# griffin-h/lightcurve_fitting

Hardware: AMD Instinct MI355X
Metric: walker-steps/sec (emcee ensemble) (higher is better)
Workload: dtype f64

## Files before the change

lightcurve_fitting_amd/csrc/lcf_hip.hip:

```cpp
#include <hip/hip_runtime.h>

#include <algorithm>
#include <chrono>
#include <cmath>
#include <cstdio>
#include <cstdlib>
#include <dlfcn.h>
#include <cstring>
#include <mutex>
#include <numeric>
#include <string>
#include <vector>

#include "lcf.h"
#include "lcf_device.h"
#include "lcf_host.h"
#include "lcf_internal.h"
#include "lcf_keys.h"

#ifndef LCF_KPRE
#define LCF_KPRE 4
#endif
#ifndef LCF_KPRE_SOLO
#define LCF_KPRE_SOLO 2
// ... 937 lines not shown
        step_serial<ND>(pb, sm, i, true, threadIdx.x, have_prev, prev_row, have_next, draws, prev_draws, g, mine, sc, nullptr,
                        coef, lprior);
}

template <int ND>
__global__ __launch_bounds__(64) void k_step(const DevProblem pb, const DevSampler sm, int have_prev, long long prev_row,
                                             int have_next, const DrawRec* __restrict__ draws,
                                             const DrawRec* __restrict__ prev_draws, long long g, int lo, int hi,
                                             double* __restrict__ coef, double* __restrict__ lprior) {
    step_body<ND>(pb, sm, blockIdx.x, have_prev, prev_row, have_next, draws, prev_draws, g, lo, hi, coef, lprior);
}

constexpr int kFusedScratch = kNCoef + 2 + kMaxDim + (kMaxDim & 1);

__device__ inline double uniform_f64(double v) {
    const long long b = __double_as_longlong(v);
    const int lo = __builtin_amdgcn_readfirstlane((int)(b & 0xffffffffLL));
    const int hi = __builtin_amdgcn_readfirstlane((int)(b >> 32));
    return __longlong_as_double(((long long)hi << 32) | (unsigned int)lo);
}

template <int ND, int VARIANT, bool THERM>
__global__ __launch_bounds__(kBlock, LCF_WAVES) void k_fused(const DevProblem pb, const DevSampler sm, int have_prev,
                                                  long long prev_row, const DrawRec* __restrict__ draws,
                                                  const DrawRec* __restrict__ prev_draws, long long g, int lo, int hi,
                                                  double* __restrict__ lprior) {
    extern __shared__ __align__(16) unsigned char smem[];
    double* exptab = reinterpret_cast<double*>(smem);
    double* red = exptab + kExpTabSize;
    double2* ltab = reinterpret_cast<double2*>(smem + kLdsHead * sizeof(double));
    const FiltDesc* fdesc = reinterpret_cast<const FiltDesc*>(ltab + pb.n_lds_tab);
    const int itab_at = pb.n_itab_lds > 0
                            ? (int)(kLdsHead * sizeof(double) + (pb.n_lds_tab + kFdD2 * pb.n_filters) * sizeof(double2)) : -1;
    double* sc = reinterpret_cast<double*>(ltab + pb.stage_d2);
    double* sq = sc + kNCoef + 2;
    const int tid = threadIdx.x;
    const int n_own = hi - lo;
    if ((int)blockIdx.x >= n_own * pb.n_parts) {
        const int k = ((int)blockIdx.x - n_own * pb.n_parts) * (kBlock / 64) + (tid >> 6);
        const int slot = k < lo ? k : k + n_own;
        if (slot < sm.n_half)
            step_serial<ND>(pb, sm, slot, true, tid & 63, have_prev, prev_row, 1, draws, prev_draws, g, false, nullptr,
                            nullptr, nullptr, nullptr);
        return;
    }
    const int part = blockIdx.x / n_own, i = lo + blockIdx.x % n_own;
    const bool reddened = pb.model == kShockCooling3;
    if (tid < 64)
        step_serial<ND>(pb, sm, i, part == 0, tid, have_prev, prev_row, 1, draws, prev_draws, g, true, sc, sq, nullptr,
                        lprior);
    else if (!reddened)
        stage_tables<VARIANT, true>(pb, exptab, ltab, 0., tid - 64, kBlock - 64);
    __syncthreads();
    if (sc[kNCoef] == -INFINITY) return;
    double cs[kNCoef];
#pragma unroll
    for (int k = 0; k < kNCoef; ++k) cs[k] = uniform_f64(sc[k]);
    if (reddened) stage_tables<VARIANT, true>(pb, exptab, ltab, cs[6], tid, kBlock);
    if (reddened) __syncthreads();
    double term;
    if constexpr (THERM)
        term = epochs_loop<VARIANT, true>(pb, part, sq, cs, ltab, fdesc, ExpTab{exptab}, tid, itab_at);
    else
        term = points_loop<VARIANT, 0, true, false>(pb, part, 0, sq, cs, nullptr, 0, ltab, fdesc, ExpTab{exptab}, nullptr,
                                                    nullptr, tid, itab_at);
    const double psum = store_part_sum(term, red, sm.part2[g & 1] + (size_t)i * part_stride(pb) + part);
    if (sm.n_peers > 0 && tid == 0) mbox_post(sm, g, i, part, part_stride(pb), psum);
}

__device__ inline unsigned long long* board_entry(unsigned long long* board, const DevSampler& sm, unsigned int tag, int wid,
                                                  int col) {
    return board + 2 * ((((size_t)(tag & (unsigned int)(sm.ring - 1)) * sm.n_walkers) + wid) * board_row_entries(sm.n_dim) + col);
}
#ifndef LCF_EARLY_POST
#define LCF_EARLY_POST 0
#endif
#ifndef LCF_EARLY_LOG
#define LCF_EARLY_LOG 1
#endif
__device__ __forceinline__ int not_hoisted(int v) {
    asm volatile("" : "+v"(v));
    return v;
}
__device__ __forceinline__ size_t board_entry_bytes(const RunUniforms& u, unsigned int tag, int wid, int col) {
    return (tag & u.ring_mask) * u.ver_bytes + ((size_t)(unsigned int)wid * u.row_bytes + 16u * (unsigned int)col);
}
__device__ __forceinline__ unsigned long long* board_entry(unsigned long long* board, const RunUniforms& u, unsigned int tag,
                                                           int wid, int col) {
    return reinterpret_cast<unsigned long long*>(reinterpret_cast<unsigned char*>(board) + board_entry_bytes(u, tag, wid, col));
}
__device__ inline unsigned int* board_progress(unsigned long long* board, const DevSampler& sm) {
    return reinterpret_cast<unsigned int*>(reinterpret_cast<unsigned char*>(board) +
                                           board_rows_bytes(sm.ring, sm.n_walkers, sm.n_dim));
}
typedef unsigned int lcf_u32x4 __attribute__((ext_vector_type(4)));
typedef int lcf_i32x4 __attribute__((ext_vector_type(4)));
template <bool AGENT>
__device__ __forceinline__ void store16_past_caches(unsigned long long* p, unsigned long long lo, unsigned long long hi) {
    const lcf_u32x4 v = {(unsigned int)lo, (unsigned int)(lo >> 32), (unsigned int)hi, (unsigned int)(hi >> 32)};
    asm volatile("global_store_dwordx4 %0, %1, off sc0 sc1" : : "v"(p), "v"(v) : "memory");
}
template <bool AGENT>
__device__ __forceinline__ void load16_past_caches(const unsigned long long* p, unsigned long long& lo, unsigned long long& hi) {
    lcf_u32x4 v;
    asm volatile("global_load_dwordx4 %0, %1, off sc0 sc1\n\ts_waitcnt vmcnt(0)" : "=v"(v) : "v"(p) : "memory");
    lo = (unsigned long long)v.x | ((unsigned long long)v.y << 32);
    hi = (unsigned long long)v.z | ((unsigned long long)v.w << 32);
}
template <bool AGENT = false>
__device__ inline void board_post_at(unsigned long long* entry, unsigned int tag, double v) {
    const unsigned long long b = (unsigned long long)__double_as_longlong(v), t = (unsigned long long)tag << 32;
    store16_past_caches<AGENT>(entry, (b & 0xffffffffull) | t, (b >> 32) | t);
}
template <bool AGENT = false>
__device__ inline void board_post(unsigned long long* board, const DevSampler& sm, unsigned int tag, int wid, int col, double v) {
    board_post_at<AGENT>(board_entry(board, sm, tag, wid, col), tag, v);
}
template <bool AGENT = false>
__device__ inline bool board_aborted_at(const unsigned int* flag) {
    return (AGENT ? __hip_atomic_load(flag, __ATOMIC_RELAXED, __HIP_MEMORY_SCOPE_AGENT)
                  : __hip_atomic_load(flag, __ATOMIC_RELAXED, __HIP_MEMORY_SCOPE_SYSTEM)) != 0u;
}
template <bool AGENT = false>
__device__ inline bool board_aborted(const DevSampler& sm) {
    return board_aborted_at<AGENT>(board_progress(sm.board, sm) + kMaxPeers);
}
__device__ inline unsigned int* board_arrivals(const DevSampler& sm) { return board_progress(sm.board, sm) + kMaxPeers + 5; }
__device__ inline void board_abort(const DevSampler& sm, unsigned int what, unsigned int a, unsigned int b, unsigned int c) {
    unsigned int* flag = board_progress(sm.board, sm) + kMaxPeers;
    if (atomicCAS_system(flag, 0u, 1u) == 0u) {
        __hip_atomic_store(flag + 1, what, __ATOMIC_RELAXED, __HIP_MEMORY_SCOPE_SYSTEM);
        __hip_atomic_store(flag + 2, a, __ATOMIC_RELAXED, __HIP_MEMORY_SCOPE_SYSTEM);
        __hip_atomic_store(flag + 3, b, __ATOMIC_RELAXED, __HIP_MEMORY_SCOPE_SYSTEM);
        __hip_atomic_store(flag + 4, c, __ATOMIC_RELAXED, __HIP_MEMORY_SCOPE_SYSTEM);
    }
    atomicOr(sm.err, 2);
    if (sm.snap_flags) sm.snap_flags[kSnapFlags + (blockIdx.x & (kSnapFlags - 1))] = 2u;
}
template <bool AGENT = false>
__device__ inline double board_take_at(const DevSampler& sm, const unsigned long long* p, unsigned int tag, int wid, int col,
                                       unsigned int arrive_goal = 0u) {
    const unsigned long long t0 = wall_clock64();
    bool resident = arrive_goal == 0u;
    for (int spin = 0;; ++spin) {
        unsigned long long a, b;
        load16_past_caches<AGENT>(p, a, b);
        if ((unsigned int)(a >> 32) == tag && (unsigned int)(b >> 32) == tag)
            return __longlong_as_double((long long)((a & 0xffffffffull) | (b << 32)));
        if ((spin & 15) == 15) {
            if (board_aborted<AGENT>(sm)) return qnan();
            if (!resident && wall_clock64() - t0 > sm.resident_ticks) {
                const unsigned int there = __hip_atomic_load(board_arrivals(sm), __ATOMIC_RELAXED, __HIP_MEMORY_SCOPE_AGENT);
                if ((int)(there - arrive_goal) < 0) {
                    board_abort(sm, 3u, tag, (unsigned int)wid, there);
                    return qnan();
                }
                resident = true;
            }
            if (wall_clock64() - t0 > sm.wait_ticks) {
                const bool was_first = !board_aborted<AGENT>(sm);
                board_abort(sm, 1u, tag, (unsigned int)wid, (unsigned int)col);
                if (was_first) {
                    unsigned int* seen = board_arrivals(sm) + 1;
                    seen[0] = (unsigned int)a;
                    seen[1] = (unsigned int)(a >> 32);
                    seen[2] = (unsigned int)b;
                    seen[3] = (unsigned int)(b >> 32);
                }
                return qnan();
            }
        }
        __builtin_amdgcn_s_sleep(1);
    }
}
template <bool AGENT = false>
__device__ inline double board_take(const DevSampler& sm, unsigned int tag, int wid, int col, unsigned int arrive_goal = 0u) {
    return board_take_at<AGENT>(sm, board_entry(sm.board, sm, tag, wid, col), tag, wid, col, arrive_goal);
}
template <bool AGENT>
// ... 109 lines not shown
    const double* cs_ = sm.X + (size_t)dr.pid * nd;
    h.got = 0.;
    if (BOARD) {
        const bool own = lane >= 16;
        const int col = own ? lane - 16 : lane;
        if (own ? col <= nd + 1 : col < nd) {
            const unsigned int tag = board_tag(G, own ? dr.wage : dr.page, g_run0);
            const int who = own ? dr.wid : dr.pid;
            h.got = board_take<BOARD == 2>(sm, tag, who, col, arrive_goal);
        }
    }
    h.lp_i = BOARD ? lane_value(h.got, 16 + nd) : sm.LP[dr.wid];
#pragma unroll
    for (int d = 0; d < kD; ++d) {
        h.x[d] = d < nd ? (BOARD ? lane_value(h.got, 16 + d) : xs[d]) : 0.;
        h.cj[d] = d < nd ? (BOARD ? lane_value(h.got, d) : cs_[d]) : 0.;
    }
    h.prior = PriorDev{0, 0, 0., 0., 0., 1.};
    if (lane < pb.n_dim && pb.has_priors) h.prior = pb.priors[lane];
}

template <int ND, int BOARD = 0, int MODEL = 0>
__device__ __forceinline__ void proposal_head(const DevProblem& pb, const DevSampler& sm, const DrawRec& dr, int lane,
                                              double* __restrict__ sc, double* __restrict__ sq, double* __restrict__ sx,
                                              const HeadRows<ND>& h) {
    constexpr int kD = ND > 0 ? ND : kMaxDim;
    const int nd = ND > 0 ? ND : sm.n_dim;
    const PriorDev my_prior = h.prior;
    double x[kD], q[kMaxDim], lq[kMaxDim];
#pragma unroll
    for (int d = 0; d < kMaxDim; ++d) q[d] = lq[d] = 0.;
    const double got = h.got;
    const double lp_i = h.lp_i;
    double arg = 1.;
#pragma unroll
    for (int d = 0; d < kD; ++d) {
        x[d] = h.x[d];
        const double cj = h.cj[d];
        q[d] = d < nd ? cj - (cj - x[d]) * dr.z : 0.;
        if (lane == d && d < pb.n_par) arg = q[d];
    }
#ifdef LCF_STAMPS
    asm volatile("s_waitcnt vmcnt(0)" ::: "memory");
#endif
    LCF_STAMP(0, 2);
    const double lg = flog(arg);
#pragma unroll
    for (int d = 0; d < kD; ++d) lq[d] = lane_value(lg, d);
    LCF_STAMP(0, 3);
    double c[kNCoef];
    walker_coefficients<MODEL>(pb, q, lq, c, MODEL ? true : pb.use_itab != 0);
    LCF_STAMP(0, 4);
    double lpr = 0.;
    if (pb.has_priors) {
        double qv = 0.;
#pragma unroll
        for (int d = 0; d < kD; ++d)
            if (lane == d) qv = q[d];
        const double mine = lane < pb.n_dim ? prior_term(my_prior, qv) : 0.;
#pragma unroll
        for (int d = 0; d < kD; ++d)
            if (d < nd) lpr += lane_value(mine, d);
    }
    const double count = BOARD ? lane_value(got, 16 + nd + 1) : 0.;
    if (lane == 0) {
#pragma unroll
        for (int k = 0; k < kNCoef; ++k) sc[k] = c[k];
        sc[kNCoef] = lpr;
#pragma unroll
        for (int d = 0; d < kD; ++d)
            if (d < nd) {
                sq[d] = q[d];
                sx[d] = x[d];
            }
        sx[kMaxDim] = lp_i;
        if (BOARD) sx[kMaxDim + 1] = count;
    }
    LCF_STAMP(0, 5);
}

struct LaneRows {
    double cj, x;
    PriorDev prior;
};

template <int ND, int BOARD>
__device__ __forceinline__ void lane_head_fetch(const DevSampler& sm, const DrawRec& dr, int lane_in, LaneRows& h, long long G,
                                                long long g_run0, unsigned int arrive_goal, const RunUniforms* ru) {
    const int nd = ND > 0 ? ND : __builtin_amdgcn_readfirstlane(ru->nd);
    const int lane = not_hoisted(lane_in);
    h.cj = h.x = 0.;
    if (lane <= nd + 1) {
        const unsigned int wtag = board_tag(G, dr.wage, g_run0), ptag = board_tag(G, dr.page, g_run0);
        const bool both = lane < nd;
        const unsigned int tag_l = both ? ptag : wtag;
        const int wid_l = both ? dr.pid : dr.wid;
        board_take_pair<BOARD == 2>(sm, board_entry(ru->board, *ru, tag_l, wid_l, lane), board_entry(ru->board, *ru, wtag, dr.wid, lane),
                                    tag_l, wtag, wid_l, dr.wid, lane, arrive_goal, h.cj, h.x);
    }
    h.prior = ru->priors[lane & (kMaxDim - 1)];
}

template <int MODEL>
__device__ __attribute__((noinline)) void cold_coefficients(const double* consts, const double* p_mem, double* c_mem, bool write) {
    static_assert(MODEL == kShockCooling, "the model whose coefficients have a branch worth moving out");
    double p[kMaxDim], lq[kMaxDim], c[kNCoef];
#pragma unroll
    for (int d = 0; d < kMaxDim; ++d) p[d] = lq[d] = 0.;
#pragma unroll
    for (int d = 0; d < 5; ++d) p[d] = p_mem[d];
#pragma unroll
    for (int d = 0; d < 4; ++d) lq[d] = flog(p[d]);
    walker_coefficients<MODEL>(ConstsView{consts, MODEL}, p, lq, c, true);
    if (write) {
#pragma unroll
        for (int k = 0; k < kNCoef; ++k) c_mem[k] = c[k];
    }
}

template <int ND, int BOARD, int MODEL, bool EARLY = false>
__device__ __forceinline__ void lane_head(const DevProblem& pb, const DrawRec& dr, int lane_in, double* __restrict__ sc,
                                          double* __restrict__ sq, double* __restrict__ sx, const LaneRows& h,
                                          const RunUniforms* ru) {
    constexpr int kD = ND > 0 ? ND : kMaxDim;
    const int nd = ND > 0 ? ND : __builtin_amdgcn_readfirstlane(ru->nd);
    const int lane = not_hoisted(lane_in);
    const int n_par = ru->n_par, n_dim = ru->n_dim, has_priors = __builtin_amdgcn_readfirstlane(ru->has_priors);
    const double cj = h.cj, x = h.x;
    const double q = lane < nd ? cj - (cj - x) * dr.z : 0.;
#ifdef LCF_STAMPS
    asm volatile("s_waitcnt vmcnt(0)" ::: "memory");
#endif
    LCF_STAMP(0, 2);
    if (lane < nd) sq[lane] = q;
    if constexpr (EARLY) __syncthreads();
    if (lane <= nd + 1) sx[lane < nd ? lane : lane - nd + kMaxDim] = x;
    const double lg = flog(lane < n_par ? q : 1.);
    double p[kMaxDim], lq[kMaxDim];
#pragma unroll
    for (int d = 0; d < kMaxDim; ++d) p[d] = lq[d] = 0.;
#pragma unroll
    for (int d = 0; d < kD; ++d) {
        p[d] = lane_value(q, d);
        lq[d] = lane_value(lg, d);
    }
    LCF_STAMP(0, 3);
    double c[kNCoef];
    bool c_stored = false;
    if constexpr (MODEL == kShockCooling) {
        const double v = p[0], M = p[1], f = p[2], R = p[3];
        if (v > 0. && M > 0. && f > 0. && R > 0. && v < 1e100 && M < 1e100 && f < 1e100 && R < 1e100) {
            walker_coefficients<MODEL, ConstsView, true>(ConstsView{ru->consts, MODEL}, p, lq, c, true);
        } else {
#pragma unroll
            for (int k = 0; k < kNCoef; ++k) c[k] = 0.;
            cold_coefficients<MODEL>(ru->consts, sq, sc, lane == 0);
            c_stored = true;
        }
    } else {
        walker_coefficients<MODEL>(ConstsView{ru->consts, MODEL ? MODEL : ru->model}, p, lq, c, MODEL ? true : pb.use_itab != 0);
    }
    LCF_STAMP(0, 4);
    double lpr = 0.;
    if (has_priors) {
        const double mine = lane < n_dim ? prior_term(h.prior, q) : 0.;
#pragma unroll
        for (int d = 0; d < kD; ++d)
            if (d < nd) lpr += lane_value(mine, d);
    }
    if (lane == 0) {
        if (!c_stored) {
#pragma unroll
            for (int k = 0; k < kNCoef; k += 2) *reinterpret_cast<double2*>(sc + k) = make_double2(c[k], c[k + 1]);
        }
        sc[kNCoef] = lpr;
    }
    LCF_STAMP(0, 5);
}

constexpr int kSoloScratch = kNCoef + 2 + 2 * (kMaxDim + (kMaxDim & 1));

template <int ND, int VARIANT, bool THERM, int NPARTS, int BOARD, int MODEL>
__device__ __forceinline__ bool solo_half_step(const DevProblem& pb, const DevProblem* __restrict__ pbp, const DevSampler& sm, long long row,
                                               const DrawRec* __restrict__ draws, const DrawRec* draws_next, long long G,
                                               long long g_run0, int i, unsigned char* smem, ColumnOperands& first_col,
                                               bool first, bool write_state, const int tid, const int run_flags = 0,
                                               const unsigned int arrive_goal = 0u, const RunUniforms* ru = nullptr) {
    constexpr bool RES = BOARD >= 2;
    double* exptab = reinterpret_cast<double*>(smem);
    double* red = exptab + kExpTabSize;
    double2* ltab = reinterpret_cast<double2*>(smem + kLdsHead * sizeof(double));
    const FiltDesc* fdesc = RES ? nullptr : reinterpret_cast<const FiltDesc*>(ltab + pb.n_lds_tab);
    int itab_at = -1;
    if constexpr (!RES)
        itab_at = pb.n_itab_lds > 0
                      ? (int)(kLdsHead * sizeof(double) + (pb.n_lds_tab + kFdD2 * pb.n_filters) * sizeof(double2)) : -1;
    double* sc = RES ? reinterpret_cast<double*>(const_cast<RunUniforms*>(ru)) - (kSoloScratch + 4)
                     : reinterpret_cast<double*>(ltab + pb.stage_d2);
    double* sq = sc + kNCoef + 2;
    double* sx = sq + kMaxDim + (kMaxDim & 1);
    int* sctl = reinterpret_cast<int*>(sc + (RES ? kNCoef + 1 : kSoloScratch + 2));
    constexpr int kGroups = NPARTS == 8 ? 4 : 2;
    constexpr int kThreads = kBlock * kGroups;
    constexpr int kD = ND > 0 ? ND : kMaxDim;
    const int nd = ND > 0 ? ND : RES ? __builtin_amdgcn_readfirstlane(ru->nd) : sm.n_dim;
    const bool reddened = !MODEL && (RES ? __builtin_amdgcn_readfirstlane(ru->model) : pb.model) == kShockCooling3;
    LCF_STAMP(0, 0);
#ifdef LCF_STAMPS
    if (tid == 0 && blockIdx.x < 1024) g_wall[((G & 1) * 1024 + blockIdx.x) * 2] = wall_clock64();
#endif
    const DrawRec dr = draws[i];
    if (BOARD == 1 && blockIdx.x == 0 && tid < sm.n_board_ranks)
        __hip_atomic_store(board_progress(sm.peer_board[tid], sm) + sm.board_rank, (unsigned int)G, __ATOMIC_RELAXED,
                           __HIP_MEMORY_SCOPE_SYSTEM);
    if (dr.wid < 0) return false;
    LCF_STAMP(0, 1);
    constexpr bool kFetch = MODEL != 0;
    constexpr bool kEarly = RES && MODEL != 0 && NPARTS <= 2 && LCF_EARLY_LOG != 0;
    constexpr int kT0 = MODEL == kShockCooling ? 4 : MODEL == kShockCooling2 ? 3 : -1;
    static_assert(!kEarly || kT0 >= 0, "a model-specialised resident kernel names the coordinate that is t_0");
    double lt_early = 0.;
    if (tid < 64) {
        if (BOARD >= 2) __builtin_amdgcn_s_setprio(3);
        if constexpr (RES) {
            LaneRows rows;
            lane_head_fetch<ND, BOARD>(sm, dr, tid, rows, G, g_run0, arrive_goal, ru);
            if (kFetch && first) fetch_column<VARIANT, MODEL>(pb, tid / kBlock, tid % kBlock, first_col);
            lane_head<ND, BOARD, MODEL, kEarly>(pb, dr, tid, sc, sq, sx, rows, ru);
        } else {
            HeadRows<ND> rows;
            head_fetch<ND, BOARD>(pb, sm, dr, tid, rows, G, g_run0, arrive_goal);
            if (kFetch && first) fetch_column<VARIANT, MODEL>(pb, tid / kBlock, tid % kBlock, first_col);
            proposal_head<ND, BOARD, MODEL>(pb, sm, dr, tid, sc, sq, sx, rows);
        }
        if (BOARD >= 2) __builtin_amdgcn_s_setprio(0);
    } else {
        if (LCF_HEAD_START > 0) __builtin_amdgcn_s_sleep(LCF_HEAD_START);
        if (kFetch && first) fetch_column<VARIANT, MODEL>(pb, tid / kBlock, tid % kBlock, first_col);
        if (BOARD >= 2) {
            if (tid >= 64 && tid < 128 && draws_next != nullptr) {
                const int* nxt = reinterpret_cast<const int*>(draws_next + i);
                int a_, b_;
                asm volatile("s_load_dword %0, %2, 0x0\n\ts_load_dword %1, %2, 0x2c\n\ts_waitcnt lgkmcnt(0)"
                             : "=&s"(a_), "=&s"(b_) : "s"(nxt) : "memory");
            }
        } else if (tid == 64 && draws_next != nullptr) {
            const volatile int* nxt = reinterpret_cast<const volatile int*>(draws_next + i);
            (void)nxt[0];
            (void)nxt[sizeof(DrawRec) / sizeof(int) - 1];
        }
        if constexpr (RES)
            if (tid == 64) sctl[0] = board_aborted_at<BOARD == 2>(ru->abort_word) ? 1 : 0;
        if constexpr (kEarly) {
            const int tid_e = not_hoisted(tid);
            const bool lean_e = __builtin_amdgcn_readfirstlane(ru->group[__builtin_amdgcn_readfirstlane(tid_e / kBlock)].lean) != 0;
            const bool mine = lean_e && first_col.have_o;
            __syncthreads();
            const double t0 = sq[kT0];
            if (mine) lt_early = tlog(first_col.t - t0);
        }
        if (!reddened && first) stage_tables<VARIANT, true>(pb, exptab, ltab, 0., tid - 64, kThreads - 64);
        LCF_STAMP(1, 11);
        if (BOARD == 1 && tid < 128) {
            const int lane = tid - 64;
            const unsigned int* progress = board_progress(sm.board, sm);
            const unsigned long long t0 = wall_clock64();
            bool abort = false;
            for (;;) {
                bool ok = true;
                if (G - 2 >= g_run0 && lane < sm.n_board_ranks)
                    ok = (int)(__hip_atomic_load(progress + lane, __ATOMIC_RELAXED, __HIP_MEMORY_SCOPE_SYSTEM) -
                               (unsigned int)(G - 1)) >= 0;
                abort = board_aborted(sm);
                if (__all(ok) || abort) break;
                if (wall_clock64() - t0 > sm.wait_ticks) {
                    board_abort(sm, 2u, (unsigned int)G, (unsigned int)__builtin_ctzll(~__ballot(ok)), 0u);
                    abort = true;
                    break;
                }
                __builtin_amdgcn_s_sleep(2);
            }
            if (lane == 0) sctl[0] = abort ? 1 : 0;
        }
    }
    __syncthreads();
    LCF_STAMP(0, 6);
    double lpr;
    lcf_i32x4 col_group = {0, 0, 0, 0}, col_itab = {0, 0, 0, 0};
    double2 col_grid = make_double2(0., 0.);
    double col_consts[5] = {0., 0., 0., 0., 0.};
    if constexpr (RES) {
        const double2 la = *reinterpret_cast<const double2*>(sc + kNCoef);
        if constexpr (MODEL != 0 && NPARTS <= 2) {
            const int group = __builtin_amdgcn_readfirstlane(not_hoisted(tid) / kBlock);
// ... 10 lines not shown
        lpr = sc[kNCoef];
    }
    double term = 0.;
    const bool excluded = lpr == -INFINITY;
    bool lean = false;
    if (MODEL != 0 && NPARTS <= 2 && !excluded) {
        const int tid_c = RES ? not_hoisted(tid) : tid;
        const int part = __builtin_amdgcn_readfirstlane(tid_c / kBlock), ltid = tid_c % kBlock;
        int c0, c1;
        if constexpr (RES) {
            c0 = __builtin_amdgcn_readfirstlane(col_group.x);
            c1 = __builtin_amdgcn_readfirstlane(col_group.y);
            lean = first_col.have_o && __builtin_amdgcn_readfirstlane(col_group.z) != 0;
        } else {
            c0 = part_entry(pb.part_col0, part);
            c1 = part_entry(pb.part_col0, part + 1);
            lean = first_col.have_o && itab_at >= 0 && c1 - c0 <= kBlock && part < pb.n_parts;
        }
        if (lean) {
            LCF_STAMP(0, 7);
            double acc = 0.;
            if (c0 + (ltid & ~63) < c1) {
                const bool live = c0 + ltid < c1;
                bool in_grid;
                if constexpr (kEarly) {
                    if (__builtin_amdgcn_readfirstlane(tid_c >> 6) == 0)
                        lt_early = tlog(first_col.t - sc[0]);
                    in_grid = lean_column<MODEL, true>(ColumnView{col_consts, col_grid.x, col_grid.y, col_itab.x, nullptr}, sc,
                                                       first_col, ExpTab{exptab}, col_itab.y, acc, lt_early);
                } else if constexpr (RES)
                    in_grid = lean_column<MODEL>(ColumnView{col_consts, col_grid.x, col_grid.y, col_itab.x, nullptr}, sc, first_col,
                                                 ExpTab{exptab}, col_itab.y, acc);
                else
                    in_grid = lean_column<MODEL>(pb, sc, first_col, ExpTab{exptab}, itab_at, acc);
                if (!in_grid)
                    acc = cold_column_with_state<VARIANT, MODEL>(pbp, sc, sq, first_col.t, min(c0 + ltid, c1 - 1), live);
                term = live ? acc : 0.;
            }
            LCF_STAMP(0, 8);
            LCF_STAMP(1, 12);
            const double ws = wave_sum(term);
            if ((tid & 63) == 0) red[tid_c >> 6] = ws;
        }
    }
    if (!excluded && !lean) {
        double cs[kNCoef];
#pragma unroll
        for (int k = 0; k < kNCoef; ++k) cs[k] = uniform_f64(sc[k]);
        if constexpr (RES) {
            fdesc = reinterpret_cast<const FiltDesc*>(ltab + pb.n_lds_tab);
            itab_at = __builtin_amdgcn_readfirstlane(ru->itab_at);
        }
        if (reddened) stage_tables<VARIANT, true>(pb, exptab, ltab, cs[6], tid, kThreads);
        const int part = tid / kBlock, ltid = tid % kBlock;
        if (reddened) __syncthreads();
        LCF_STAMP(0, 7);
        if (NPARTS > 2) {
#pragma unroll 1
            for (int pp = part; pp < pb.n_parts; pp += kGroups) {
                term = epochs_loop<VARIANT, true, kFetch, MODEL, true>(pb, pp, sq, cs, ltab, fdesc, ExpTab{exptab}, ltid, itab_at,
                                                                       first_col, pp == part, pbp, sc);
                const double ws = wave_sum(term);
                if ((tid & 63) == 0) red[4 * pp + (ltid >> 6)] = ws;
            }
        } else {
            if (part < pb.n_parts)
                term = epochs_loop<VARIANT, true, kFetch, MODEL, true>(pb, part, sq, cs, ltab, fdesc, ExpTab{exptab}, ltid, itab_at,
                                                                       first_col, true, pbp, sc);
            LCF_STAMP(0, 8);
            LCF_STAMP(1, 12);
            const double ws = wave_sum(term);
            if ((tid & 63) == 0) red[tid >> 6] = ws;
        }
    }
    size_t entry_early = 0;
    if constexpr (RES && LCF_EARLY_POST != 0)
        if (tid < 64) entry_early = board_entry_bytes(*ru, (unsigned int)(G + 1), dr.wid, not_hoisted(tid));
    __syncthreads();
    LCF_STAMP(0, 9);
    if (BOARD) {
        if (tid >= 64) return false;
        if (BOARD >= 2) __builtin_amdgcn_s_setprio(3);
        if constexpr (RES) {
            const double2* red2 = reinterpret_cast<const double2*>(red);
            const double2 lc = *reinterpret_cast<const double2*>(sx + kMaxDim);
            const int col = not_hoisted(tid);
            const int mine = col < nd ? col : 0;
            const double q_mine = sq[mine], x_mine = sx[mine];
            const double sum0 = ru->sum0;
            const unsigned int tag = (unsigned int)(G + 1);
            const size_t entry = LCF_EARLY_POST != 0 ? entry_early : board_entry_bytes(*ru, tag, dr.wid, col);
            unsigned char* const own_board = reinterpret_cast<unsigned char*>(ru->board);
            double sum = sum0;
            if (NPARTS <= 2) {
                const int n_parts = ru->n_parts;
                const double2 a0 = red2[0], a1 = red2[1], b0 = red2[2], b1 = red2[3];
                const double s1 = sum + ((a0.x + a0.y) + (a1.x + a1.y));
                sum = n_parts > 0 ? s1 : sum;
                const double s2 = sum + ((b0.x + b0.y) + (b1.x + b1.y));
                sum = n_parts > 1 ? s2 : sum;
            } else {
                const int n_parts = __builtin_amdgcn_readfirstlane(ru->n_parts);
                for (int k = 0; k < n_parts; ++k) sum += (red2[2 * k].x + red2[2 * k].y) + (red2[2 * k + 1].x + red2[2 * k + 1].y);
            }
            const double scored = lpr - 0.5 * sum;
            const double nlp = excluded ? -INFINITY : scored;
            const double lp_i = lc.x;
            const bool ok = (dr.zl + nlp - lp_i) > dr.lnu;
            const double count = lc.y + (ok ? 1. : 0.);
            if (tid <= nd + 1) {
                const double v = tid < nd ? (ok ? q_mine : x_mine) : tid == nd ? (ok ? nlp : lp_i) : count;
                if (BOARD == 2) {
                    board_post_at<true>(reinterpret_cast<unsigned long long*>(own_board + entry), tag, v);
                } else {
#pragma unroll
                    for (int r = 0; r < kMaxPeers; ++r)
                        if (r < sm.n_board_ranks)
                            board_post_at(reinterpret_cast<unsigned long long*>(reinterpret_cast<unsigned char*>(sm.peer_board[r]) + entry),
                                          tag, v);
                }
                if (BOARD == 2 && write_state) {
                    if (tid < nd)
                        ru->X[(size_t)dr.wid * nd + tid] = v;
                    else if (tid == nd)
                        ru->LP[dr.wid] = v;
                    else
                        ru->nacc[dr.wid] = (long long)v;
                    unsigned long long* const snap = ru->snap_out;
                    if (snap) {
                        const size_t nw = ru->n_walkers;
                        if (tid < nd) snap[1 + (size_t)dr.wid * nd + tid] = (unsigned long long)__double_as_longlong(v);
                        else if (tid == nd) snap[1 + nw * nd + dr.wid] = (unsigned long long)__double_as_longlong(v);
                        else snap[1 + nw * nd + nw + dr.wid] = (unsigned long long)(long long)v;
                    }
                }
                if (BOARD == 2 && (run_flags & kRunStoreChain)) {
                    const size_t at = (size_t)row * ru->n_walkers + dr.wid;
                    if (tid < nd) ru->chain[at * nd + tid] = v;
                    else if (tid == nd) ru->chain_lp[at] = v;
                }
            }
            if (tid == 0 && nlp != nlp) {
                atomicOr(sm.err, 1);
                if (BOARD == 2 && sm.snap_flags) sm.snap_flags[blockIdx.x & (kSnapFlags - 1)] = 1u;
            }
            __builtin_amdgcn_s_setprio(0);
            LCF_STAMP(0, 10);
            return false;
        }
        double nlp = -INFINITY;
        if (!excluded) {
            double sum = pb.use_sigma ? 0. : pb.log_norm_const;
            for (int k = 0; k < pb.n_parts; ++k) sum += (red[4 * k] + red[4 * k + 1]) + (red[4 * k + 2] + red[4 * k + 3]);
            nlp = lpr - 0.5 * sum;
        }
        const double lp_i = sx[kMaxDim];
        const bool ok = (dr.zl + nlp - lp_i) > dr.lnu;
        const double count = sx[kMaxDim + 1] + (ok ? 1. : 0.);
        if (tid <= nd + 1) {
            const double v = tid < nd ? (ok ? sq[tid] : sx[tid]) : tid == nd ? (ok ? nlp : lp_i) : count;
            if (BOARD == 2) {
                board_post<true>(sm.board, sm, (unsigned int)(G + 1), dr.wid, tid, v);
            } else {
#pragma unroll
                for (int r = 0; r < kMaxPeers; ++r)
                    if (r < sm.n_board_ranks) board_post(sm.peer_board[r], sm, (unsigned int)(G + 1), dr.wid, tid, v);
            }
            if (BOARD == 1 || (BOARD == 2 && write_state)) {
                const bool to_out = BOARD == 2 && !(run_flags & kRunFlip);
                double* X = to_out ? sm.X_out : sm.X;
                double* LP = to_out ? sm.LP_out : sm.LP;
                long long* nacc = to_out ? sm.nacc_out : sm.nacc;
                if (tid < nd)
                    X[(size_t)dr.wid * nd + tid] = v;
                else if (tid == nd)
                    LP[dr.wid] = v;
                else
                    nacc[dr.wid] = (long long)v;
                if (BOARD == 2 && sm.snap_out) {
                    const size_t nw = sm.n_walkers;
                    if (tid < nd) sm.snap_out[1 + (size_t)dr.wid * nd + tid] = (unsigned long long)__double_as_longlong(v);
                    else if (tid == nd) sm.snap_out[1 + nw * nd + dr.wid] = (unsigned long long)__double_as_longlong(v);
                    else sm.snap_out[1 + nw * nd + nw + dr.wid] = (unsigned long long)(long long)v;
                }
            }
            if (BOARD == 2 && (run_flags & kRunStoreChain)) {
                if (tid < nd) sm.chain[((size_t)row * sm.n_walkers + dr.wid) * nd + tid] = v;
                else if (tid == nd) sm.chain_lp[(size_t)row * sm.n_walkers + dr.wid] = v;
            }
        }
        if (tid == 0 && nlp != nlp) {
            atomicOr(sm.err, 1);
            if (BOARD == 2 && sm.snap_flags) sm.snap_flags[blockIdx.x & (kSnapFlags - 1)] = 1u;
        }
        if (BOARD >= 2) __builtin_amdgcn_s_setprio(0);
        LCF_STAMP(0, 10);
        return false;
    }
    if (tid != 0) return false;
    double nlp = -INFINITY;
    if (!excluded) {
        double sum = pb.use_sigma ? 0. : pb.log_norm_const;
        for (int k = 0; k < pb.n_parts; ++k) sum += (red[4 * k] + red[4 * k + 1]) + (red[4 * k + 2] + red[4 * k + 3]);
        nlp = lpr - 0.5 * sum;
    }
    const double lp_i = sx[kMaxDim];
    const bool ok = (dr.zl + nlp - lp_i) > dr.lnu;
    if (nlp != nlp) atomicOr(sm.err, 1);
    if (ok) {
#pragma unroll
        for (int d = 0; d < kD; ++d)
            if (d < nd) sm.X[(size_t)dr.wid * nd + d] = sq[d];
        sm.LP[dr.wid] = nlp;
        atomicAdd(reinterpret_cast<unsigned long long*>(&sm.nacc[dr.wid]), 1ull);
    }
    if (sm.store_chain) {
        double* crow = sm.chain + ((size_t)row * sm.n_walkers + dr.wid) * nd;
#pragma unroll
        for (int d = 0; d < kD; ++d)
            if (d < nd) crow[d] = ok ? sq[d] : sx[d];
// ... 64 lines not shown
        const int d = lane - 32;
        const bool has = d < pb.n_dim && pb.has_priors;
        const PriorDev* pr = pb.priors + (has ? d : 0);
        ru->priors[d].kind = has ? pr->kind : 0;
        ru->priors[d].pad = 0;
        ru->priors[d].p_min = has ? pr->p_min : 0.;
        ru->priors[d].p_max = has ? pr->p_max : 0.;
        ru->priors[d].mean = has ? pr->mean : 0.;
        ru->priors[d].stddev = has ? pr->stddev : 1.;
    }
}

template <int ND, int VARIANT, bool THERM, int NPARTS, int MODEL, bool RANKS = false>
__global__ __launch_bounds__(kBlock * (NPARTS == 8 ? 4 : 2), LCF_WAVES)
void k_solo_run(const DevProblem* __restrict__ pbp, const DevSampler* __restrict__ smp, long long rel0,
                const DrawRec* __restrict__ draws0, long long g_run0, int n_hs, long long state_from, int n_wg, int run_flags,
                unsigned int arrive_goal, int slot_lo, int n_slots, long long need_progress) {
    extern __shared__ __align__(16) unsigned char smem[];
    ColumnOperands first_col;
    typedef const DevProblem __attribute__((address_space(4)))* ProblemPtr;
    typedef const DevSampler __attribute__((address_space(4)))* SamplerPtr;
    const DevProblem& pb = *(const DevProblem*)(ProblemPtr)pbp;
    const DevSampler& sm = *(const DevSampler*)(SamplerPtr)smp;
    constexpr int kBoard = RANKS ? 3 : 2;
    bool first = true;
    RunUniforms* const ru = reinterpret_cast<RunUniforms*>(smem + kLdsHead * sizeof(double) + (size_t)pb.stage_d2 * sizeof(double2) +
                                                           (kSoloScratch + 4) * sizeof(double));
    if (threadIdx.x >= 64 && threadIdx.x < 128) fill_run_uniforms(pb, sm, ru, run_flags, RANKS, threadIdx.x - 64);
    if (!RANKS) __syncthreads();
    if (threadIdx.x == 0) __hip_atomic_fetch_add(board_arrivals(sm), 1u, __ATOMIC_RELAXED, __HIP_MEMORY_SCOPE_AGENT);
    if (RANKS) {
        __shared__ int s_abort;
        if (blockIdx.x == 0 && threadIdx.x < sm.n_board_ranks)
            __hip_atomic_store(board_progress(sm.peer_board[threadIdx.x], sm) + sm.board_rank, (unsigned int)(g_run0 + rel0),
                               __ATOMIC_RELAXED, __HIP_MEMORY_SCOPE_SYSTEM);
        if (threadIdx.x < 64) {
            bool abort = false;
            if (need_progress > 0) {
                const int lane = threadIdx.x;
                const unsigned int* progress = board_progress(sm.board, sm);
                const unsigned long long t0 = wall_clock64();
                for (;;) {
                    bool ok = true;
                    if (lane < sm.n_board_ranks)
                        ok = (int)(__hip_atomic_load(progress + lane, __ATOMIC_RELAXED, __HIP_MEMORY_SCOPE_SYSTEM) -
                                   (unsigned int)need_progress) >= 0;
                    abort = board_aborted(sm);
                    if (__all(ok) || abort) break;
                    if (wall_clock64() - t0 > sm.wait_ticks) {
                        board_abort(sm, 2u, (unsigned int)(g_run0 + rel0), (unsigned int)__builtin_ctzll(~__ballot(ok)),
                                    (unsigned int)need_progress);
                        abort = true;
                        break;
                    }
                    __builtin_amdgcn_s_sleep(8);
                }
            }
            if (threadIdx.x == 0) s_abort = abort ? 1 : 0;
        }
        __syncthreads();
        if (s_abort != 0) return;
    }
    if (!RANKS && rel0 == 0) {
        const int nd = ND > 0 ? ND : sm.n_dim;
        const int col = threadIdx.x & 31;
        const bool flip = (run_flags & kRunFlip) != 0;
        const double* X = flip ? sm.X_out : sm.X;
        const double* LP = flip ? sm.LP_out : sm.LP;
        const long long* nacc = flip ? sm.nacc_out : sm.nacc;
        for (int w = blockIdx.x * (int)(blockDim.x / 32) + (int)(threadIdx.x / 32); w < sm.n_walkers;
             w += n_wg * (int)(blockDim.x / 32))
            if (col <= nd + 1) {
                const double v = col < nd ? X[(size_t)w * nd + col] : col == nd ? LP[w] : (double)nacc[w];
                board_post<true>(sm.board, sm, (unsigned int)g_run0, w, col, v);
            }
    }
    const int slot_end = slot_lo + n_slots;
    const int n_half = sm.n_half;
#pragma unroll 1
    for (int h = 0; h < n_hs; ++h) {
        const DrawRec* draws = draws0 + (size_t)h * n_half;
#pragma unroll 1
        for (int i = slot_lo + blockIdx.x; i < slot_end; i += n_wg) {
            if (draws[i].wid < 0) continue;
            const bool more = i + n_wg < slot_end;
            const DrawRec* hint = more ? draws + n_wg : h + 1 < n_hs ? draws + n_half + (slot_lo + (int)blockIdx.x - i) : nullptr;
            const int tid = threadIdx.x;
            if (solo_half_step<ND, VARIANT, THERM, NPARTS, kBoard, MODEL>(pb, pbp, sm, (rel0 + h) >> 1, draws, hint,
                                                                          g_run0 + rel0 + h, g_run0, i, smem, first_col, first,
                                                                          rel0 + h >= state_from, tid, run_flags, arrive_goal, ru))
                return;
            first = false;
        }
    }
}

template <class T>
__global__ void k_put_image(T* __restrict__ dst, const T src) {
    if (threadIdx.x == 0 && blockIdx.x == 0) *dst = src;
}

struct MultiItem {
    DevProblem pb;
    DevSampler sm;
    const DrawRec* draws[2];
    long long blk_first, blk_steps;
    double* coef;
    double* lprior;
    long long g_run0;
    int flip, itab_extra;
    unsigned int arrive0, pad;
};

__device__ inline const DrawRec* item_rows(const MultiItem& it, long long rel) {
    const long long k = rel / 2;
    const long long b = k < it.blk_first ? 0 : 1 + (k - it.blk_first) / it.blk_steps;
    const long long k0 = b == 0 ? 0 : it.blk_first + (b - 1) * it.blk_steps;
    return it.draws[b & 1] + (size_t)(rel - 2 * k0) * it.sm.n_half;
}

template <int ND>
__global__ __launch_bounds__(64) void k_step_multi(const MultiItem* __restrict__ items, int have_prev, long long prev_row,
                                                   int have_next, long long rel, long long g) {
    const MultiItem& it = items[blockIdx.y];
    const int nh = it.sm.n_half;
    if ((int)blockIdx.x >= nh) return;
    step_body<ND>(it.pb, it.sm, blockIdx.x, have_prev, prev_row, have_next,
                  have_next ? item_rows(it, rel) : nullptr, have_prev ? item_rows(it, rel - 1) : nullptr,
                  g, 0, nh, it.coef, it.lprior);
}

template <int VARIANT, bool LDS_TAB, bool THERM>
__global__ __launch_bounds__(kBlock) void k_points_multi(const MultiItem* __restrict__ items, int parity) {
    const MultiItem& it = items[blockIdx.y];
    const int nh = it.sm.n_half;
    if ((int)blockIdx.x >= nh * it.pb.n_parts) return;
    points_body<VARIANT, 0, LDS_TAB, THERM>(it.pb, blockIdx.x, 0, nh, it.sm.Q[parity], it.coef, it.lprior, nullptr,
                                            it.sm.part2[parity], nullptr);
}

constexpr int kPopScratch = kSoloScratch + 6;
constexpr int kPopMaxParts = 4;
#ifndef LCF_POP_RUN_GROUP
#define LCF_POP_RUN_GROUP 4
#endif
constexpr int kPopRunGroup = LCF_POP_RUN_GROUP;

#ifndef LCF_POP_WAVES
#define LCF_POP_WAVES LCF_WAVES
#endif
template <int ND, int VARIANT, int GROUP, int MODEL = 0>
__global__ __launch_bounds__(64 * GROUP, LCF_POP_WAVES) void k_pop(const MultiItem* __restrict__ items, long long rel) {
    extern __shared__ __align__(16) unsigned char smem[];
    typedef const MultiItem __attribute__((address_space(4)))* ItemPtr;
    const ItemPtr itp = (ItemPtr)(items + blockIdx.y);
    const MultiItem& it = *(const MultiItem*)itp;
    const DevProblem& pb = it.pb;
    const DevSampler& sm = it.sm;
    constexpr int kThreads = 64 * GROUP;
    const int nh = sm.n_half, slot0 = blockIdx.x * GROUP;
    if (slot0 >= nh) return;
    double* exptab = reinterpret_cast<double*>(smem);
    double2* ltab = reinterpret_cast<double2*>(smem + kLdsHead * sizeof(double));
    const FiltDesc* fdesc = reinterpret_cast<const FiltDesc*>(ltab + pb.n_lds_tab);
    const int itab_at = pb.n_itab_lds > 0
                            ? (int)(kLdsHead * sizeof(double) + (pb.n_lds_tab + kFdD2 * pb.n_filters) * sizeof(double2)) : -1;
    double* scratch = reinterpret_cast<double*>(ltab + pb.stage_d2);
    double* red = scratch + GROUP * kPopScratch;
    constexpr int kD = ND > 0 ? ND : kMaxDim;
    const int nd = ND > 0 ? ND : sm.n_dim;
    const int tid = threadIdx.x, lane = tid & 63, wave = __builtin_amdgcn_readfirstlane(tid >> 6);
    {
        double* sc = scratch + wave * kPopScratch;
// ... 2014 lines not shown
```

Before: 104.7 million.

## Load draw records via scalar loads and batch commit-stage operand reads

Reads each draw record through the constant address space so its fields land in scalar registers, then passes that record into the half-step instead of reloading it. The commit stage's LDS reads (partial sums, proposal, position, log-post, uniforms) are issued as one inline-asm batch with a single wait, and the record's zl/lnu/wid are refetched with scalar loads. The lane-head fetch preloads the board geometry and prior counts in one place. The aim is to shorten the serial latency chain on the per-step critical path. The hand-written asm relies on fixed struct offsets and LDS layout and adds maintenance risk.

```diff
diff --git a/lightcurve_fitting_amd/csrc/lcf_hip.hip b/lightcurve_fitting_amd/csrc/lcf_hip.hip
--- a/lightcurve_fitting_amd/csrc/lcf_hip.hip
+++ b/lightcurve_fitting_amd/csrc/lcf_hip.hip
@@ -1043,8 +1043,103 @@
     asm volatile("" : "+v"(v));
     return v;
 }
+#ifndef LCF_SCALAR_DRAW
+#define LCF_SCALAR_DRAW 1
+#endif
+#ifndef LCF_BATCH_HEAD
+#define LCF_BATCH_HEAD 1
+#endif
+#ifndef LCF_BATCH_COMMIT
+#define LCF_BATCH_COMMIT 1
+#endif
+typedef unsigned int lcf_u32x4 __attribute__((ext_vector_type(4)));
+typedef int lcf_i32x4 __attribute__((ext_vector_type(4)));
+template <bool SCALAR>
+__device__ __forceinline__ DrawRec draw_record(const DrawRec* p) {
+    if constexpr (SCALAR) {
+        typedef const DrawRec __attribute__((address_space(4)))* DrawPtr;
+        const DrawPtr c = (DrawPtr)p;
+        DrawRec r;
+        r.wid = c->wid, r.pid = c->pid, r.wprev = c->wprev, r.pprev = c->pprev;
+        r.z = c->z, r.zl = c->zl, r.lnu = c->lnu;
+        r.wage = c->wage, r.page = c->page;
+        int z_lo = __double2loint(r.z), z_hi = __double2hiint(r.z);
+        asm volatile("" : "+s"(r.wid), "+s"(r.pid), "+s"(z_lo), "+s"(z_hi), "+s"(r.wage), "+s"(r.page));
+        r.z = __hiloint2double(z_hi, z_lo);
+        return r;
+    } else {
+        return *p;
+    }
+}
+__device__ __forceinline__ unsigned int lds_offset(const void* p) {
+    typedef const __attribute__((address_space(3))) unsigned char* LdsBytes;
+    return (unsigned int)(__SIZE_TYPE__)(LdsBytes)p;
+}
+__device__ __forceinline__ double f64_of(unsigned int lo, unsigned int hi) { return __hiloint2double((int)hi, (int)lo); }
+constexpr int kScProposal = (kNCoef + 2) * 8;
+constexpr int kScPosition = kScProposal + (kMaxDim + (kMaxDim & 1)) * 8;
+constexpr int kScLogPost = kScPosition + kMaxDim * 8;
+constexpr int kScUniforms = (kNCoef + 2 + 2 * (kMaxDim + (kMaxDim & 1)) + 4) * 8;
+static_assert(kScLogPost % 16 == 0 && kScUniforms % 16 == 0, "16-byte reads");
+static_assert(offsetof(RunUniforms, ring_mask) == 8 && offsetof(RunUniforms, row_bytes) == 12 && offsetof(RunUniforms, ver_bytes) == 16 &&
+              offsetof(RunUniforms, sum0) == 32 && offsetof(RunUniforms, n_parts) == 40,
+              "the groups the batch below reads with one instruction each");
+struct CommitOperands {
+    lcf_u32x4 a0, a1, b0, b1, lc, sums, geo;
+    double ver_bytes, q_mine, x_mine;
+    lcf_u32x4 zl_lnu;
+    int wid;
+};
+template <bool RECORD>
+__device__ __forceinline__ void commit_batch(unsigned int red_at, unsigned int sc_at, unsigned int mine_at, const void* rec,
+                                             CommitOperands& c) {
+    if constexpr (RECORD)
+        asm volatile("ds_read_b128 %0, %12\n\t"
+                     "ds_read_b128 %1, %12 offset:16\n\t"
+                     "ds_read_b128 %2, %12 offset:32\n\t"
+                     "ds_read_b128 %3, %12 offset:48\n\t"
+                     "ds_read_b128 %4, %13 offset:%16\n\t"
+                     "ds_read_b128 %5, %13 offset:%17\n\t"
+                     "ds_read_b128 %6, %13 offset:%18\n\t"
+                     "ds_read_b64 %7, %13 offset:%19\n\t"
+                     "ds_read_b64 %8, %14 offset:%20\n\t"
+                     "ds_read_b64 %9, %14 offset:%21\n\t"
+                     "s_load_dwordx4 %10, %15, 0x18\n\t"
+                     "s_load_dword %11, %15, 0x0\n\t"
+                     "s_waitcnt lgkmcnt(0)"
+                     : "=&v"(c.a0), "=&v"(c.a1), "=&v"(c.b0), "=&v"(c.b1), "=&v"(c.lc), "=&v"(c.sums), "=&v"(c.geo), "=&v"(c.ver_bytes),
+                       "=&v"(c.q_mine), "=&v"(c.x_mine), "=&s"(c.zl_lnu), "=&s"(c.wid)
+                     : "v"(red_at), "v"(sc_at), "v"(mine_at), "s"(rec), "n"(kScLogPost), "n"(kScUniforms + 32), "n"(kScUniforms),
+                       "n"(kScUniforms + 16), "n"(kScProposal), "n"(kScPosition)
+                     : "memory");
+    else
+        asm volatile("ds_read_b128 %0, %10\n\t"
+                     "ds_read_b128 %1, %10 offset:16\n\t"
+                     "ds_read_b128 %2, %10 offset:32\n\t"
+                     "ds_read_b128 %3, %10 offset:48\n\t"
+                     "ds_read_b128 %4, %11 offset:%13\n\t"
+                     "ds_read_b128 %5, %11 offset:%14\n\t"
+                     "ds_read_b128 %6, %11 offset:%15\n\t"
+                     "ds_read_b64 %7, %11 offset:%16\n\t"
+                     "ds_read_b64 %8, %12 offset:%17\n\t"
+                     "ds_read_b64 %9, %12 offset:%18\n\t"
+                     "s_waitcnt lgkmcnt(0)"
+                     : "=&v"(c.a0), "=&v"(c.a1), "=&v"(c.b0), "=&v"(c.b1), "=&v"(c.lc), "=&v"(c.sums), "=&v"(c.geo), "=&v"(c.ver_bytes),
+                       "=&v"(c.q_mine), "=&v"(c.x_mine)
+                     : "v"(red_at), "v"(sc_at), "v"(mine_at), "n"(kScLogPost), "n"(kScUniforms + 32), "n"(kScUniforms),
+                       "n"(kScUniforms + 16), "n"(kScProposal), "n"(kScPosition)
+                     : "memory");
+}
+__device__ __forceinline__ void record_reload(const void* rec, lcf_u32x4& zl_lnu, int& wid) {
+    asm volatile("s_nop 4\n\ts_load_dwordx4 %0, %2, 0x18\n\ts_load_dword %1, %2, 0x0\n\ts_waitcnt lgkmcnt(0)"
+                 : "=&s"(zl_lnu), "=&s"(wid) : "s"(rec) : "memory");
+}
+__device__ __forceinline__ size_t board_entry_bytes(unsigned int ring_mask, unsigned long long ver_bytes, unsigned int row_bytes,
+                                                    unsigned int tag, int wid, int col) {
+    return (tag & ring_mask) * ver_bytes + ((size_t)(unsigned int)wid * row_bytes + 16u * (unsigned int)col);
+}
 __device__ __forceinline__ size_t board_entry_bytes(const RunUniforms& u, unsigned int tag, int wid, int col) {
-    return (tag & u.ring_mask) * u.ver_bytes + ((size_t)(unsigned int)wid * u.row_bytes + 16u * (unsigned int)col);
+    return board_entry_bytes(u.ring_mask, u.ver_bytes, u.row_bytes, tag, wid, col);
 }
 __device__ __forceinline__ unsigned long long* board_entry(unsigned long long* board, const RunUniforms& u, unsigned int tag,
                                                            int wid, int col) {
@@ -1054,8 +1149,6 @@
     return reinterpret_cast<unsigned int*>(reinterpret_cast<unsigned char*>(board) +
                                            board_rows_bytes(sm.ring, sm.n_walkers, sm.n_dim));
 }
-typedef unsigned int lcf_u32x4 __attribute__((ext_vector_type(4)));
-typedef int lcf_i32x4 __attribute__((ext_vector_type(4)));
 template <bool AGENT>
 __device__ __forceinline__ void store16_past_caches(unsigned long long* p, unsigned long long lo, unsigned long long hi) {
     const lcf_u32x4 v = {(unsigned int)lo, (unsigned int)(lo >> 32), (unsigned int)hi, (unsigned int)(hi >> 32)};
@@ -1331,6 +1424,7 @@
 struct LaneRows {
     double cj, x;
     PriorDev prior;
+    int n_par, n_dim, has_priors;
 };
 
 template <int ND, int BOARD>
@@ -1339,13 +1433,24 @@
     const int nd = ND > 0 ? ND : __builtin_amdgcn_readfirstlane(ru->nd);
     const int lane = not_hoisted(lane_in);
     h.cj = h.x = 0.;
+    h.n_par = h.n_dim = h.has_priors = 0;
+    unsigned char* board = reinterpret_cast<unsigned char*>(ru->board);
+    unsigned int ring_mask = ru->ring_mask, row_bytes = ru->row_bytes;
+    unsigned long long ver_bytes = ru->ver_bytes;
+    if constexpr (LCF_BATCH_HEAD != 0) {
+        h.n_par = ru->n_par, h.n_dim = ru->n_dim, h.has_priors = ru->has_priors;
+        asm volatile("" : "+v"(board), "+v"(ring_mask), "+v"(row_bytes), "+v"(ver_bytes), "+v"(h.n_par), "+v"(h.n_dim), "+v"(h.has_priors));
+    }
     if (lane <= nd + 1) {
         const unsigned int wtag = board_tag(G, dr.wage, g_run0), ptag = board_tag(G, dr.page, g_run0);
         const bool both = lane < nd;
         const unsigned int tag_l = both ? ptag : wtag;
         const int wid_l = both ? dr.pid : dr.wid;
-        board_take_pair<BOARD == 2>(sm, board_entry(ru->board, *ru, tag_l, wid_l, lane), board_entry(ru->board, *ru, wtag, dr.wid, lane),
-                                    tag_l, wtag, wid_l, dr.wid, lane, arrive_goal, h.cj, h.x);
+        const unsigned long long* const pa =
+            reinterpret_cast<const unsigned long long*>(board + board_entry_bytes(ring_mask, ver_bytes, row_bytes, tag_l, wid_l, lane));
+        const unsigned long long* const pw =
+            reinterpret_cast<const unsigned long long*>(board + board_entry_bytes(ring_mask, ver_bytes, row_bytes, wtag, dr.wid, lane));
+        board_take_pair<BOARD == 2>(sm, pa, pw, tag_l, wtag, wid_l, dr.wid, lane, arrive_goal, h.cj, h.x);
     }
     h.prior = ru->priors[lane & (kMaxDim - 1)];
 }
@@ -1374,7 +1479,8 @@
     constexpr int kD = ND > 0 ? ND : kMaxDim;
     const int nd = ND > 0 ? ND : __builtin_amdgcn_readfirstlane(ru->nd);
     const int lane = not_hoisted(lane_in);
-    const int n_par = ru->n_par, n_dim = ru->n_dim, has_priors = __builtin_amdgcn_readfirstlane(ru->has_priors);
+    const int n_par = LCF_BATCH_HEAD != 0 ? h.n_par : ru->n_par, n_dim = LCF_BATCH_HEAD != 0 ? h.n_dim : ru->n_dim;
+    const int has_priors = __builtin_amdgcn_readfirstlane(LCF_BATCH_HEAD != 0 ? h.has_priors : ru->has_priors);
     const double cj = h.cj, x = h.x;
     const double q = lane < nd ? cj - (cj - x) * dr.z : 0.;
 #ifdef LCF_STAMPS
@@ -1434,7 +1540,8 @@
                                                const DrawRec* __restrict__ draws, const DrawRec* draws_next, long long G,
                                                long long g_run0, int i, unsigned char* smem, ColumnOperands& first_col,
                                                bool first, bool write_state, const int tid, const int run_flags = 0,
-                                               const unsigned int arrive_goal = 0u, const RunUniforms* ru = nullptr) {
+                                               const unsigned int arrive_goal = 0u, const RunUniforms* ru = nullptr,
+                                               const DrawRec* held = nullptr) {
     constexpr bool RES = BOARD >= 2;
     double* exptab = reinterpret_cast<double*>(smem);
     double* red = exptab + kExpTabSize;
@@ -1458,7 +1565,7 @@
 #ifdef LCF_STAMPS
     if (tid == 0 && blockIdx.x < 1024) g_wall[((G & 1) * 1024 + blockIdx.x) * 2] = wall_clock64();
 #endif
-    const DrawRec dr = draws[i];
+    const DrawRec dr = held != nullptr ? *held : draws[i];
     if (BOARD == 1 && blockIdx.x == 0 && tid < sm.n_board_ranks)
         __hip_atomic_store(board_progress(sm.peer_board[tid], sm) + sm.board_rank, (unsigned int)G, __ATOMIC_RELAXED,
                            __HIP_MEMORY_SCOPE_SYSTEM);
@@ -1635,32 +1742,59 @@
         if (tid >= 64) return false;
         if (BOARD >= 2) __builtin_amdgcn_s_setprio(3);
         if constexpr (RES) {
-            const double2* red2 = reinterpret_cast<const double2*>(red);
-            const double2 lc = *reinterpret_cast<const double2*>(sx + kMaxDim);
             const int col = not_hoisted(tid);
             const int mine = col < nd ? col : 0;
-            const double q_mine = sq[mine], x_mine = sx[mine];
-            const double sum0 = ru->sum0;
             const unsigned int tag = (unsigned int)(G + 1);
-            const size_t entry = LCF_EARLY_POST != 0 ? entry_early : board_entry_bytes(*ru, tag, dr.wid, col);
-            unsigned char* const own_board = reinterpret_cast<unsigned char*>(ru->board);
-            double sum = sum0;
-            if (NPARTS <= 2) {
-                const int n_parts = ru->n_parts;
-                const double2 a0 = red2[0], a1 = red2[1], b0 = red2[2], b1 = red2[3];
-                const double s1 = sum + ((a0.x + a0.y) + (a1.x + a1.y));
+            constexpr bool kRecord = LCF_SCALAR_DRAW != 0;
+            int wid = dr.wid;
+            double zl = dr.zl, lnu = dr.lnu, sum, lp_i, count0, q_mine, x_mine;
+            size_t entry;
+            unsigned char* own_board;
+            if constexpr (NPARTS <= 2 && LCF_BATCH_COMMIT != 0) {
+                const unsigned int sc_at = lds_offset(sc);
+                CommitOperands c;
+                commit_batch<kRecord>(lds_offset(red), sc_at, sc_at + 8u * (unsigned int)mine, draws + i, c);
+                if constexpr (kRecord) wid = c.wid, zl = f64_of(c.zl_lnu.x, c.zl_lnu.y), lnu = f64_of(c.zl_lnu.z, c.zl_lnu.w);
+                entry = (tag & c.geo.z) * (unsigned long long)__double_as_longlong(c.ver_bytes) +
+                        ((size_t)(unsigned int)wid * c.geo.w + 16u * (unsigned int)col);
+                own_board = reinterpret_cast<unsigned char*>((size_t)c.geo.x | ((size_t)c.geo.y << 32));
+                sum = f64_of(c.sums.x, c.sums.y);
+                const int n_parts = (int)c.sums.z;
+                const double s1 = sum + ((f64_of(c.a0.x, c.a0.y) + f64_of(c.a0.z, c.a0.w)) + (f64_of(c.a1.x, c.a1.y) + f64_of(c.a1.z, c.a1.w)));
                 sum = n_parts > 0 ? s1 : sum;
-                const double s2 = sum + ((b0.x + b0.y) + (b1.x + b1.y));
+                const double s2 = sum + ((f64_of(c.b0.x, c.b0.y) + f64_of(c.b0.z, c.b0.w)) + (f64_of(c.b1.x, c.b1.y) + f64_of(c.b1.z, c.b1.w)));
                 sum = n_parts > 1 ? s2 : sum;
+                lp_i = f64_of(c.lc.x, c.lc.y), count0 = f64_of(c.lc.z, c.lc.w);
+                q_mine = c.q_mine, x_mine = c.x_mine;
             } else {
-                const int n_parts = __builtin_amdgcn_readfirstlane(ru->n_parts);
-                for (int k = 0; k < n_parts; ++k) sum += (red2[2 * k].x + red2[2 * k].y) + (red2[2 * k + 1].x + red2[2 * k + 1].y);
+                if constexpr (kRecord) {
+                    lcf_u32x4 r;
+                    record_reload(draws + i, r, wid);
+                    zl = f64_of(r.x, r.y), lnu = f64_of(r.z, r.w);
+                }
+                const double2* red2 = reinterpret_cast<const double2*>(red);
+                const double2 lc = *reinterpret_cast<const double2*>(sx + kMaxDim);
+                q_mine = sq[mine], x_mine = sx[mine];
+                entry = LCF_EARLY_POST != 0 ? entry_early : board_entry_bytes(*ru, tag, wid, col);
+                own_board = reinterpret_cast<unsigned char*>(ru->board);
+                sum = ru->sum0;
+                if (NPARTS <= 2) {
+                    const int n_parts = ru->n_parts;
+                    const double2 a0 = red2[0], a1 = red2[1], b0 = red2[2], b1 = red2[3];
+                    const double s1 = sum + ((a0.x + a0.y) + (a1.x + a1.y));
+                    sum = n_parts > 0 ? s1 : sum;
+                    const double s2 = sum + ((b0.x + b0.y) + (b1.x + b1.y));
+                    sum = n_parts > 1 ? s2 : sum;
+                } else {
+                    const int n_parts = __builtin_amdgcn_readfirstlane(ru->n_parts);
+                    for (int k = 0; k < n_parts; ++k) sum += (red2[2 * k].x + red2[2 * k].y) + (red2[2 * k + 1].x + red2[2 * k + 1].y);
+                }
+                lp_i = lc.x, count0 = lc.y;
             }
             const double scored = lpr - 0.5 * sum;
             const double nlp = excluded ? -INFINITY : scored;
-            const double lp_i = lc.x;
-            const bool ok = (dr.zl + nlp - lp_i) > dr.lnu;
-            const double count = lc.y + (ok ? 1. : 0.);
+            const bool ok = (zl + nlp - lp_i) > lnu;
+            const double count = count0 + (ok ? 1. : 0.);
             if (tid <= nd + 1) {
                 const double v = tid < nd ? (ok ? q_mine : x_mine) : tid == nd ? (ok ? nlp : lp_i) : count;
                 if (BOARD == 2) {
@@ -1674,21 +1808,21 @@
                 }
                 if (BOARD == 2 && write_state) {
                     if (tid < nd)
-                        ru->X[(size_t)dr.wid * nd + tid] = v;
+                        ru->X[(size_t)wid * nd + tid] = v;
                     else if (tid == nd)
-                        ru->LP[dr.wid] = v;
+                        ru->LP[wid] = v;
                     else
-                        ru->nacc[dr.wid] = (long long)v;
+                        ru->nacc[wid] = (long long)v;
                     unsigned long long* const snap = ru->snap_out;
                     if (snap) {
                         const size_t nw = ru->n_walkers;
-                        if (tid < nd) snap[1 + (size_t)dr.wid * nd + tid] = (unsigned long long)__double_as_longlong(v);
-                        else if (tid == nd) snap[1 + nw * nd + dr.wid] = (unsigned long long)__double_as_longlong(v);
-                        else snap[1 + nw * nd + nw + dr.wid] = (unsigned long long)(long long)v;
+                        if (tid < nd) snap[1 + (size_t)wid * nd + tid] = (unsigned long long)__double_as_longlong(v);
+                        else if (tid == nd) snap[1 + nw * nd + wid] = (unsigned long long)__double_as_longlong(v);
+                        else snap[1 + nw * nd + nw + wid] = (unsigned long long)(long long)v;
                     }
                 }
                 if (BOARD == 2 && (run_flags & kRunStoreChain)) {
-                    const size_t at = (size_t)row * ru->n_walkers + dr.wid;
+                    const size_t at = (size_t)row * ru->n_walkers + wid;
                     if (tid < nd) ru->chain[at * nd + tid] = v;
                     else if (tid == nd) ru->chain_lp[at] = v;
                 }
@@ -1919,13 +2053,15 @@
         const DrawRec* draws = draws0 + (size_t)h * n_half;
 #pragma unroll 1
         for (int i = slot_lo + blockIdx.x; i < slot_end; i += n_wg) {
-            if (draws[i].wid < 0) continue;
+            const DrawRec rec = draw_record<LCF_SCALAR_DRAW != 0>(draws + i);
+            if (rec.wid < 0) continue;
             const bool more = i + n_wg < slot_end;
             const DrawRec* hint = more ? draws + n_wg : h + 1 < n_hs ? draws + n_half + (slot_lo + (int)blockIdx.x - i) : nullptr;
             const int tid = threadIdx.x;
             if (solo_half_step<ND, VARIANT, THERM, NPARTS, kBoard, MODEL>(pb, pbp, sm, (rel0 + h) >> 1, draws, hint,
                                                                           g_run0 + rel0 + h, g_run0, i, smem, first_col, first,
-                                                                          rel0 + h >= state_from, tid, run_flags, arrive_goal, ru))
+                                                                          rel0 + h >= state_from, tid, run_flags, arrive_goal, ru,
+                                                                          LCF_SCALAR_DRAW != 0 ? &rec : nullptr))
                 return;
             first = false;
         }
```

After: 106.9 million, median of 6. 2.2% higher.
